# deezer/musicFPaugment

Hardware: AMD Instinct MI355X
Metric: 8s/8kHz clips/sec (STFT+UNet+peak-pick) (higher is better)
Workload: dtype bf16x3 (fp32 operands split into bf16 hi+lo, fp32 accumulate); 1 GPU; STFT(512/256,f64) -> UNet(1,1) eval forward (bf16x3 MFMA, formula weights) -> Audfprint peak-pick; 8 s / 8 kHz clips, 257x251 spectrograms; parallelism=clip-sharded x1, no data-path collective

## Files before the change

musicfpaugment_amd/csrc/unet_wd16.hip:

```cpp
#include "mfpa_common.h"
#include "mfpa_conv_tile.h"
#include "mfpa_unet_args.h"

namespace {

using namespace mfpa_tile;
using mfpa_unet::ConvArgs;

constexpr int KC = 32;

constexpr int wd16_bn(int wmw) { return 32 * (8 / wmw); }
constexpr bool wd16_persist(bool rows, int wmw, bool side, bool plain) { return wmw == 4 || (!rows && !side) || plain; }
template <int PH, int PW, bool IN16>
struct Wd16Lds {
  static constexpr int THREADS = 512;
  static constexpr int SPP = IN16 ? KC / 8 : KC / 4;
  static constexpr int HPW = PW + 2, HPH = PH + 2, HP = HPW * HPH;
  static constexpr int A_F4 = (HP * SPP + THREADS - 1) / THREADS;
  static constexpr int HPS = A_F4 * (THREADS / SPP);
  static constexpr int PLANE = ((HPS * 16 + 255) / 256) * 256;
  static constexpr int HLS = 4 * PLANE + 256;
  static constexpr int STAGE = 2 * HLS;
  static constexpr int TBL = 2 * A_F4 * THREADS;
  static constexpr int TBL_BYTES = 2 * ((HP * (KC / 4) + THREADS - 1) / THREADS) * THREADS * (int)sizeof(unsigned);
  static constexpr int RED = 2 * 256;
  static constexpr int epi_floats(int wmw) { return 2 * wd16_bn(wmw) + 64; }
  static constexpr int fixed_bytes(int wmw) { return 2 * STAGE + TBL_BYTES + epi_floats(wmw) * (int)sizeof(float); }
  __host__ __device__ static constexpr int plane_off(int hl, int kg) { return hl * HLS + kg * PLANE + (kg >> 1) * 128; }
  static_assert(TBL * (int)sizeof(unsigned) <= TBL_BYTES, "the kernel's table fits the launcher's");
};
static_assert(Wd16Lds<8, 32, false>::fixed_bytes(2) == 125184 && Wd16Lds<16, 16, false>::fixed_bytes(2) == 125184 &&
              Wd16Lds<8, 32, true>::fixed_bytes(2) == 125184 && Wd16Lds<16, 16, true>::fixed_bytes(2) == 125184, "LDS of the 128-channel tiles");
static_assert(Wd16Lds<8, 32, false>::fixed_bytes(4) == 124672 && Wd16Lds<8, 32, true>::fixed_bytes(4) == 124672, "LDS of the 64-channel tiles");


template <int CTRL>
__device__ __forceinline__ float dpp_row_add(float v) {
  return v + __int_as_float(__builtin_amdgcn_update_dpp(0, __float_as_int(v), CTRL, 0xf, 0xf, false));
}

template <int PH, int PW, bool ROWS, int WMW = 2, bool SIDE = false, bool PLAIN = false, bool IN16 = false, bool AFF16 = false>
__global__ __launch_bounds__(512, 1) void conv_wd16_kernel(ConvArgs a) {
  static_assert(!IN16 || PLAIN, "a bf16 source feeds the plain-bf16 products");
  using G = Wd16Lds<PH, PW, IN16>;
  constexpr int SPP = G::SPP, HPW = G::HPW, HP = G::HP, A_F4 = G::A_F4, HLS = G::HLS, STAGE = G::STAGE, TBL = G::TBL;
  constexpr int ESZ = IN16 ? 2 : 4;
  constexpr int THREADS = G::THREADS, BN = wd16_bn(WMW), WPXW = 256 / WMW, TAPS = 9;
  static_assert((WMW == 2 || WMW == 4) && (!ROWS || WMW == 2), "wave grid");
  constexpr int BM = PH * PW;
  static_assert(BM == 256 && (PW == 32 || PW == 16), "two waves of 128 pixels: eight 16-pixel tiles each");
  constexpr int PT = WPXW / 16;
  static_assert(A_F4 <= TAPS - 3, "one halo staging slot per tap, taps 2 .. 7");

  extern __shared__ __attribute__((aligned(16))) char smem[];
  const int tid = threadIdx.x, lane = tid & 63, wave = tid >> 6;
  const int wm = wave % WMW, wn = __builtin_amdgcn_readfirstlane(wave / WMW);
  const int p = lane & 15, g = lane >> 4;

  constexpr bool PERSIST = wd16_persist(ROWS, WMW, SIDE, PLAIN);
  const int n0 = blockIdx.y * BN;
  const int Cin = a.C0 + a.C1;
  const int nchunks = Cin / KC;
  const int ntiles = a.tiles_x * a.tiles_y * a.B;

  const int aq = tid % SPP;
  unsigned* const aoffs0 = reinterpret_cast<unsigned*>(smem + 2 * STAGE);
#pragma unroll
  for (int it = 0; it < A_F4; ++it) {
    const int pix = tid / SPP + it * (THREADS / SPP);
    const int py = pix / HPW - 1, px = pix % HPW - 1;
    aoffs0[it * THREADS + tid] = (unsigned)((py * a.W + px) * a.C0 + (KC / SPP) * aq) * (unsigned)ESZ;
    aoffs0[(A_F4 + it) * THREADS + tid] = (unsigned)(((py - a.oy1) * a.W1 + (px - a.ox1)) * a.C1 + (KC / SPP) * aq) * (unsigned)ESZ;
  }
  const unsigned clip0 = (unsigned)a.H * (unsigned)a.W * (unsigned)a.C0 * (unsigned)ESZ, clip1 = (unsigned)a.H1 * (unsigned)a.W1 * (unsigned)a.C1 * (unsigned)ESZ;
  struct Tile { int b, y0, x0p; unsigned ain; unsigned t0, t1; };
  auto make_tile = [&](int t) __attribute__((always_inline)) {
    Tile T;
    int bx = __builtin_amdgcn_readfirstlane(t);
    const int tx = bx % a.tiles_x; bx /= a.tiles_x;
    const int ty = bx % a.tiles_y; bx /= a.tiles_y;
    T.b = bx; T.y0 = ty * PH; T.x0p = tx * PW; T.ain = 0;
    T.t0 = (unsigned)((T.y0 * a.W + T.x0p) * a.C0) * (unsigned)ESZ;
    T.t1 = (unsigned)((T.y0 * a.W1 + T.x0p) * a.C1) * (unsigned)ESZ;
#pragma unroll
    for (int it = 0; it < A_F4; ++it) {
      const int pix = tid / SPP + it * (THREADS / SPP);
      const int gy = T.y0 + pix / HPW - 1, gx = T.x0p + pix % HPW - 1;
      const bool in = pix < HP && gy >= 0 && gy < a.H && gx >= 0 && gx < a.W;
      const int y1 = gy - a.oy1, x1 = gx - a.ox1;
      const bool in1 = in && y1 >= 0 && y1 < a.H1 && x1 >= 0 && x1 < a.W1;
      T.ain |= (in ? 1u : 0u) << it | (in1 ? 1u : 0u) << (8 + it);
    }
    return T;
  };
  auto clip_rsrc = [&](const float* base, int b, unsigned clip_bytes) __attribute__((always_inline)) {
    const char* pb = reinterpret_cast<const char*>(base) + (size_t)b * clip_bytes;
    return __builtin_amdgcn_make_buffer_rsrc(const_cast<char*>(pb), 0, base != nullptr ? (int)clip_bytes : 0, 0x00020000);
  };
  int tile = blockIdx.x;
  Tile S = make_tile(tile);
  int eb = S.b, ey0 = S.y0, ex0p = S.x0p;
  float* aff = reinterpret_cast<float*>(smem + 2 * STAGE + TBL * sizeof(unsigned));
  if (a.in_scale0 != nullptr) {
    for (int i = tid; i < a.C0; i += THREADS) {
      aff[i] = a.in_scale0[i];
      aff[a.C0 + i] = a.in_shift0[i];
    }
    __syncthreads();
  }
  float* const epi = aff + (a.in_scale0 ? 2 * a.C0 : 0) + (a.w1x1 ? G::RED : 0);
  for (int i = tid; i < BN; i += THREADS) {
    epi[i] = a.scale ? a.scale[n0 + i] : 1.f;
    epi[BN + i] = a.shift ? a.shift[n0 + i] : 0.f;
  }
  if (a.w1x1 != nullptr && tid < 64) epi[2 * BN + tid] = a.w1x1[tid];
  constexpr int AHALF = (A_F4 + 1) / 2, AREGS = ROWS ? AHALF : A_F4;
  f32x4 areg[AREGS];
  auto load_a_range = [&](int chunk, auto FIRST, auto COUNT) __attribute__((always_inline)) {
    constexpr int first = decltype(FIRST)::value, count = decltype(COUNT)::value;
    const int c0 = chunk * KC;
    const bool from0 = c0 < a.C0;
    const auto rs = clip_rsrc(from0 ? a.x0 : a.x1, S.b, from0 ? clip0 : clip1);
    const unsigned toff = from0 ? S.t0 + (unsigned)c0 * (unsigned)ESZ : S.t1 + (unsigned)(c0 - a.C0) * (unsigned)ESZ;
    const unsigned* ao = aoffs0 + (from0 ? 0 : A_F4 * THREADS) + tid;
#pragma unroll
    for (int it = first; it < first + count && it < A_F4; ++it)
      areg[it % AREGS] = __builtin_bit_cast(f32x4, __builtin_amdgcn_raw_buffer_load_b128(rs, (int)(ao[it * THREADS] + toff), 0, 0));
  };
  auto load_a = [&](int chunk) __attribute__((always_inline)) {
    load_a_range(chunk, std::integral_constant<int, 0>{}, std::integral_constant<int, AREGS>{});
  };
  auto preload_offsets = [&](int chunk) __attribute__((always_inline)) {
    const unsigned* ao = aoffs0 + (chunk * KC < a.C0 ? 0 : A_F4 * THREADS) + tid;
#pragma unroll
    for (int it = 0; it < A_F4; ++it) areg[it % AREGS][0] = __uint_as_float(ao[it * THREADS]);
  };
  auto load_a_pre = [&](int chunk) __attribute__((always_inline)) {
    const int c0 = chunk * KC;
    const bool from0 = c0 < a.C0;
    const auto rs = clip_rsrc(from0 ? a.x0 : a.x1, S.b, from0 ? clip0 : clip1);
    const unsigned toff = from0 ? S.t0 + (unsigned)c0 * (unsigned)ESZ : S.t1 + (unsigned)(c0 - a.C0) * (unsigned)ESZ;
#pragma unroll
    for (int it = 0; it < A_F4; ++it)
      areg[it % AREGS] = __builtin_bit_cast(f32x4, __builtin_amdgcn_raw_buffer_load_b128(rs, (int)(__float_as_uint(areg[it % AREGS][0]) + toff), 0, 0));
  };
  auto split_slot = [&](auto IT, int chunk, char* stage) __attribute__((always_inline)) {
    constexpr int it = decltype(IT)::value;
    const int pix = tid / SPP + it * (THREADS / SPP);
    const int c0 = chunk * KC;
    const bool inside = (S.ain >> ((c0 < a.C0 ? 0 : 8) + it)) & 1u;
    f32x4 v = areg[it % AREGS];
    if (!inside) v = f32x4{0.f, 0.f, 0.f, 0.f};
    if constexpr (IN16) {
      if (AFF16 && a.in_scale0 != nullptr && c0 < a.C0 && inside) {
        float f[8];
#pragma unroll
        for (int k = 0; k < 4; ++k) {
          const unsigned u = __float_as_uint(v[k]);
          f[2 * k] = __uint_as_float(u << 16);
          f[2 * k + 1] = __uint_as_float(u & 0xffff0000u);
        }
        const float* scp = aff + c0 + 8 * aq;
        const float* shp = aff + a.C0 + c0 + 8 * aq;
        const f32x4 sc0 = *reinterpret_cast<const f32x4*>(scp), sc1 = *reinterpret_cast<const f32x4*>(scp + 4);
        const f32x4 sh0 = *reinterpret_cast<const f32x4*>(shp), sh1 = *reinterpret_cast<const f32x4*>(shp + 4);
#pragma unroll
        for (int k = 0; k < 8; ++k) {
          const float y = f[k] * (k < 4 ? sc0[k & 3] : sc1[k & 3]) + (k < 4 ? sh0[k & 3] : sh1[k & 3]);
          f[k] = y > 0.f ? y : 0.f;
        }
        if (a.drop_thresh) {
          const int gy = S.y0 + pix / HPW - 1, gx = S.x0p + pix % HPW - 1;
          const unsigned long long e0 = (((unsigned long long)S.b * a.H + gy) * a.W + gx) * a.C0 + c0 + 8 * aq;
#pragma unroll
          for (int k = 0; k < 8; ++k) f[k] = mfpa_keep(a.drop_seed, a.drop_thresh, e0 + k) ? f[k] * a.drop_scale : 0.f;
        }
#pragma unroll
        for (int k = 0; k < 4; ++k) {
          bf16x2 h2;
          h2[0] = (__bf16)f[2 * k];
          h2[1] = (__bf16)f[2 * k + 1];
          v[k] = __builtin_bit_cast(float, h2);
        }
      }
      *reinterpret_cast<f32x4*>(stage + G::plane_off(0, aq) + pix * 16) = v;
      if constexpr (SIDE && AFF16) {
        const int py = pix / HPW, px = pix % HPW;
        if (a.x0_bf16 != nullptr && c0 < a.C0 && inside && py >= 1 && py <= PH && px >= 1 && px <= PW && blockIdx.y == 0) {
          const size_t e = (size_t)S.b * a.H * a.W * a.C0 + ((aoffs0[it * THREADS + tid] + S.t0) >> 1) + c0;
          *reinterpret_cast<f32x4*>(a.x0_bf16 + e) = v;
        }
      }
      return;
    }
    if (a.in_scale0 != nullptr && c0 < a.C0 && inside) {
      const f32x4 sc = *reinterpret_cast<const f32x4*>(aff + c0 + 4 * aq);
      const f32x4 sh = *reinterpret_cast<const f32x4*>(aff + a.C0 + c0 + 4 * aq);
      v = v * sc + sh;
#pragma unroll
      for (int k = 0; k < 4; ++k) v[k] = v[k] > 0.f ? v[k] : 0.f;
      if (a.drop_thresh) {
        const int gy = S.y0 + pix / HPW - 1, gx = S.x0p + pix % HPW - 1;
        const unsigned long long e0 = (((unsigned long long)S.b * a.H + gy) * a.W + gx) * a.C0 + c0 + 4 * aq;
#pragma unroll
        for (int k = 0; k < 4; ++k) v[k] = mfpa_keep(a.drop_seed, a.drop_thresh, e0 + k) ? v[k] * a.drop_scale : 0.f;
      }
    }
    bf16x4 hi, lo;
#pragma unroll
    for (int k = 0; k < 4; ++k) {
      hi[k] = (__bf16)v[k];
      lo[k] = (__bf16)(v[k] - (float)hi[k]);
    }
    char* at = stage + G::plane_off(0, aq >> 1) + pix * 16 + 8 * (aq & 1);
    *reinterpret_cast<bf16x4*>(at) = hi;
    if constexpr (!PLAIN) *reinterpret_cast<bf16x4*>(at + HLS) = lo;
    if constexpr (SIDE) {
      const int py = pix / HPW, px = pix % HPW;
      const bool interior = inside && py >= 1 && py <= PH && px >= 1 && px <= PW && blockIdx.y == 0;
      if (a.x0_bf16 != nullptr && c0 < a.C0 && interior) {
        const size_t e = (size_t)S.b * a.H * a.W * a.C0 + ((aoffs0[it * THREADS + tid] + S.t0) >> 2) + c0;
        *reinterpret_cast<bf16x4*>(a.x0_bf16 + e) = hi;
      }
      if (a.x1_bf16 != nullptr && c0 >= a.C0 && interior) {
        const size_t e = (size_t)S.b * a.H1 * a.W1 * a.C1 + ((aoffs0[(A_F4 + it) * THREADS + tid] + S.t1) >> 2) + (c0 - a.C0);
        *reinterpret_cast<bf16x4*>(a.x1_bf16 + e) = hi;
      }
    }
  };

  bf16x8 wq[3][2][2];
  auto w_frag = [&](int tap, int chunk) __attribute__((always_inline)) {
    return reinterpret_cast<const char*>(a.w) +
           ((((size_t)tap * nchunks + chunk) * (size_t)(a.Cout / 16) + (size_t)(n0 / 16 + 2 * wn)) << 11) + lane * 16;
  };
  auto load_w = [&](int chunk, int tap, auto SLOT) __attribute__((always_inline)) {
    constexpr int slot = decltype(SLOT)::value;
    const char* wb = w_frag(tap, chunk);
    wq[slot][0][0] = *reinterpret_cast<const bf16x8*>(wb);
    if constexpr (!PLAIN) wq[slot][0][1] = *reinterpret_cast<const bf16x8*>(wb + 1024);
    wq[slot][1][0] = *reinterpret_cast<const bf16x8*>(wb + 2048);
    if constexpr (!PLAIN) wq[slot][1][1] = *reinterpret_cast<const bf16x8*>(wb + 3072);
  };

  struct XFrags { bf16x8 h[4], l[4]; };
  XFrags fx0, fx1;
  const int xbase = (((wm * WPXW + p) / PW) * HPW + ((wm * WPXW + p) % PW)) * 16 + G::plane_off(0, g);
  auto tile_disp = [](int pt) { return (PW == 32) ? ((pt >> 1) * HPW + (pt & 1) * 16) * 16 : pt * HPW * 16; };
  auto read_x = [&](XFrags& f, const char* stage, int tap_off, int half) __attribute__((always_inline)) {
#pragma unroll
    for (int i = 0; i < 4; ++i) {
      const char* r = stage + xbase + tile_disp(4 * half + i) + tap_off;
      if constexpr (!PLAIN) f.l[i] = *reinterpret_cast<const bf16x8*>(r + HLS);
      f.h[i] = *reinterpret_cast<const bf16x8*>(r);
    }
  };
  floatx4 acc[2][PT];
#pragma unroll
  for (int ct = 0; ct < 2; ++ct)
#pragma unroll
    for (int pt = 0; pt < PT; ++pt) acc[ct][pt] = floatx4{0.f, 0.f, 0.f, 0.f};
  auto mfma_half = [&](const XFrags& f, const bf16x8 (&w)[2][2], int half) __attribute__((always_inline)) {
    if constexpr (!PLAIN) {
#pragma unroll
    for (int ct = 0; ct < 2; ++ct)
#pragma unroll
      for (int i = 0; i < 4; ++i) acc[ct][4 * half + i] = __builtin_amdgcn_mfma_f32_16x16x32_bf16(w[ct][1], f.h[i], acc[ct][4 * half + i], 0, 0, 0);
#pragma unroll
    for (int ct = 0; ct < 2; ++ct)
#pragma unroll
      for (int i = 0; i < 4; ++i) acc[ct][4 * half + i] = __builtin_amdgcn_mfma_f32_16x16x32_bf16(w[ct][0], f.l[i], acc[ct][4 * half + i], 0, 0, 0);
    }
#pragma unroll
    for (int ct = 0; ct < 2; ++ct)
#pragma unroll
      for (int i = 0; i < 4; ++i) acc[ct][4 * half + i] = __builtin_amdgcn_mfma_f32_16x16x32_bf16(w[ct][0], f.h[i], acc[ct][4 * half + i], 0, 0, 0);
  };
  using S0 = std::integral_constant<int, 0>;
  using S1 = std::integral_constant<int, 1>;
  constexpr int N_R = PLAIN ? 4 : 8, N_M = PLAIN ? 8 : 24;
  constexpr int N_W = PLAIN ? 2 : 4;
  auto tap_body = [&](auto TAP, int chunk) __attribute__((always_inline)) {
    constexpr int tap = decltype(TAP)::value;
    constexpr int ntap = (tap + 1) % TAPS;
    constexpr int tap_off = ((tap / 3) * HPW + (tap % 3)) * 16, ntap_off = ((ntap / 3) * HPW + (ntap % 3)) * 16;
    const int chunk_n = chunk + 1 < nchunks ? chunk + 1 : (PERSIST ? 0 : chunk);
    const char* cur = smem + (chunk & 1) * STAGE;
    const char* nxt = (tap == TAPS - 1) ? smem + ((chunk + 1) & 1) * STAGE : cur;
    read_x(fx1, cur, tap_off, 1);
    mfma_half(fx0, wq[tap % 3], 0);
    load_w((tap + 2 >= TAPS) ? chunk_n : chunk, (tap + 2) % TAPS, std::integral_constant<int, (tap + 2) % 3>{});
    pin_reads<N_M - 1, N_R>();
    constexpr int used_a = pin_read_slots(N_M - 1, N_R);
    __builtin_amdgcn_sched_group_barrier(0x008, 1, 0);
    __builtin_amdgcn_sched_group_barrier(0x020, N_W, 0);
    if constexpr (N_M - used_a - 1 > 0) __builtin_amdgcn_sched_group_barrier(0x008, N_M - used_a - 1, 0);
    __builtin_amdgcn_sched_barrier(0);
    if (tap == TAPS - 1) {
      __syncthreads();
      __builtin_amdgcn_sched_barrier(0);
    }
    if (tap == 0) load_a_pre(chunk_n);
    if (tap == TAPS - 1) preload_offsets(PERSIST ? (chunk + 2 < nchunks ? chunk + 2 : chunk + 1 < nchunks ? 0 : 1 < nchunks ? 1 : 0)
                                                 : (chunk + 2 < nchunks ? chunk + 2 : chunk + 1 < nchunks ? chunk + 1 : chunk));
    read_x(fx0, nxt, ntap_off, 0);
    mfma_half(fx1, wq[tap % 3], 1);
    if constexpr (tap >= 2 && tap - 2 < A_F4) {
      split_slot(std::integral_constant<int, tap - 2>{}, chunk_n, smem + ((chunk + 1) & 1) * STAGE);
#pragma unroll
      for (int i = 0; i < N_R; ++i) {
        __builtin_amdgcn_sched_group_barrier(0x008, 1, 0);
        __builtin_amdgcn_sched_group_barrier(0x100, 1, 0);
        __builtin_amdgcn_sched_group_barrier(0x002, 2, 0);
      }
#pragma unroll
      for (int i = 0; i < 2; ++i) {
        __builtin_amdgcn_sched_group_barrier(0x008, 2, 0);
        __builtin_amdgcn_sched_group_barrier(0x002, 4, 0);
        __builtin_amdgcn_sched_group_barrier(0x200, 1, 0);
      }
      if constexpr (N_M - N_R - 4 > 0) __builtin_amdgcn_sched_group_barrier(0x008, N_M - N_R - 4, 0);
    } else {
      pin_reads<N_M, N_R>();
      if constexpr (N_M - pin_read_slots(N_M, N_R) > 0) __builtin_amdgcn_sched_group_barrier(0x008, N_M - pin_read_slots(N_M, N_R), 0);
    }
    __builtin_amdgcn_sched_barrier(0);
  };

  auto tap_body4 = [&](auto TAP, auto PAR, int chunk) __attribute__((always_inline)) {
    constexpr int tap = decltype(TAP)::value, par = (decltype(PAR)::value + tap) & 1;
    constexpr int ntap = (tap + 1) % TAPS;
    constexpr int ntap_off = ((ntap / 3) * HPW + (ntap % 3)) * 16;
    const int chunk_n = chunk + 1 < nchunks ? chunk + 1 : 0;
    const char* cur = smem + (chunk & 1) * STAGE;
    const char* nxt = (tap == TAPS - 1) ? smem + ((chunk + 1) & 1) * STAGE : cur;
    if (tap == TAPS - 1) {
      __syncthreads();
      __builtin_amdgcn_sched_barrier(0);
    }
    if (tap == 0) load_a_pre(chunk_n);
    if (tap == TAPS - 1) preload_offsets(chunk + 2 < nchunks ? chunk + 2 : chunk + 1 < nchunks ? 0 : 1 < nchunks ? 1 : 0);
    read_x(par ? fx0 : fx1, nxt, ntap_off, 0);
    mfma_half(par ? fx1 : fx0, wq[tap % 3], 0);
    load_w((tap + 2 >= TAPS) ? chunk_n : chunk, (tap + 2) % TAPS, std::integral_constant<int, (tap + 2) % 3>{});
    if constexpr (tap >= 2 && tap - 2 < A_F4) {
      split_slot(std::integral_constant<int, tap - 2>{}, chunk_n, smem + ((chunk + 1) & 1) * STAGE);
#pragma unroll
      for (int i = 0; i < N_R; ++i) {
        __builtin_amdgcn_sched_group_barrier(0x008, 1, 0);
        __builtin_amdgcn_sched_group_barrier(0x100, 1, 0);
        __builtin_amdgcn_sched_group_barrier(0x002, 2, 0);
      }
#pragma unroll
      for (int i = 0; i < N_W; ++i) {
        if constexpr (!PLAIN) __builtin_amdgcn_sched_group_barrier(0x008, 1, 0);
        __builtin_amdgcn_sched_group_barrier(0x020, 1, 0);
        __builtin_amdgcn_sched_group_barrier(0x002, 2, 0);
      }
#pragma unroll
      for (int i = 0; i < 2; ++i) {
        __builtin_amdgcn_sched_group_barrier(0x008, 2, 0);
        __builtin_amdgcn_sched_group_barrier(0x002, 4, 0);
        __builtin_amdgcn_sched_group_barrier(0x200, 1, 0);
      }
      if constexpr (N_M - N_R - 8 > 0) __builtin_amdgcn_sched_group_barrier(0x008, N_M - N_R - 8, 0);
    } else {
#pragma unroll
      for (int i = 0; i < N_R; ++i) {
        __builtin_amdgcn_sched_group_barrier(0x008, 1, 0);
        __builtin_amdgcn_sched_group_barrier(0x100, 1, 0);
      }
#pragma unroll
      for (int i = 0; i < N_W; ++i) {
        __builtin_amdgcn_sched_group_barrier(0x008, 1, 0);
        __builtin_amdgcn_sched_group_barrier(0x020, 1, 0);
      }
      if constexpr (N_M - N_R - N_W > 0) __builtin_amdgcn_sched_group_barrier(0x008, N_M - N_R - N_W, 0);
    }
    __builtin_amdgcn_sched_barrier(0);
  };

  constexpr int R = BM / 2 / PW, HV = PW / 16;
  bf16x8 wr[2][3][2][2];
  constexpr int NU = (R + 2) * HV, NB = (PW == 32) ? 4 : 5;
  static_assert(NU % NB == 0, "static ring indices");
  auto load_wr1 = [&](int chunk, auto DX, auto PAR, auto DY) __attribute__((always_inline)) {
    constexpr int dx = decltype(DX)::value, par = decltype(PAR)::value, dy = decltype(DY)::value;
    const char* wb = w_frag(dy * 3 + dx, chunk);
    wr[par][dy][0][0] = *reinterpret_cast<const bf16x8*>(wb);
    if constexpr (!PLAIN) wr[par][dy][0][1] = *reinterpret_cast<const bf16x8*>(wb + 1024);
    wr[par][dy][1][0] = *reinterpret_cast<const bf16x8*>(wb + 2048);
    if constexpr (!PLAIN) wr[par][dy][1][1] = *reinterpret_cast<const bf16x8*>(wb + 3072);
  };
  struct XUnit { bf16x8 h, l; };
  XUnit xu[NB];
  auto read_unit = [&](XUnit& f, const char* stage, int u, int dx) __attribute__((always_inline)) {
    const char* r = stage + xbase + ((u / HV) * HPW + (u % HV) * 16 + dx) * 16;
    if constexpr (!PLAIN) f.l = *reinterpret_cast<const bf16x8*>(r + HLS);
    f.h = *reinterpret_cast<const bf16x8*>(r);
  };
  auto mfma_unit = [&](auto U, const XUnit& f, auto PAR) __attribute__((always_inline)) {
    constexpr int h = decltype(U)::value / HV, hv = decltype(U)::value % HV, par = decltype(PAR)::value;
#pragma unroll
    for (int term = PLAIN ? 2 : 0; term < 3; ++term)
#pragma unroll
      for (int dy = 0; dy < 3; ++dy) {
        if (h - dy < 0 || h - dy >= R) continue;
#pragma unroll
        for (int ct = 0; ct < 2; ++ct) {
          floatx4& c = acc[ct][(h - dy) * HV + hv];
          c = __builtin_amdgcn_mfma_f32_16x16x32_bf16(wr[par][dy][ct][term == 0 ? 1 : 0], term == 1 ? f.l : f.h, c, 0, 0, 0);
        }
      }
  };
  auto unit_mfmas = [](int u) { const int h = u / HV; int n = 0; for (int dy = 0; dy < 3; ++dy) n += (h - dy >= 0 && h - dy < R) ? 1 : 0; return n * (PLAIN ? 2 : 6); };
  constexpr int BARU = NU - NB + 1;
  constexpr int SA = NU / 2, SB = BARU - AHALF;
  static_assert(SA + AHALF < NU && SB >= 0, "staging schedule");
  auto unit_step = [&](auto U, auto DX, auto PAR, int chunk) __attribute__((always_inline)) {
    constexpr int u = decltype(U)::value, dx = decltype(DX)::value, par = decltype(PAR)::value;
    constexpr int n_m = unit_mfmas(u);
    const int chunk_n = chunk + 1 < nchunks ? chunk + 1 : (PERSIST ? 0 : chunk);
    const char* cur = smem + (chunk & 1) * STAGE;
    char* nxs = smem + ((chunk + 1) & 1) * STAGE;
    if constexpr (u == BARU && dx == 2) {
      __syncthreads();
      __builtin_amdgcn_sched_barrier(0);
    }
    constexpr int pu = u + NB - 1;
    if constexpr (pu < NU) read_unit(xu[pu % NB], cur, pu, dx);
    else read_unit(xu[pu % NB], dx == 2 ? nxs : cur, pu - NU, (dx + 1) % 3);
    mfma_unit(U, xu[u % NB], PAR);
    constexpr int split_it = dx == 1 ? u - SA : dx == 2 ? AHALF + u - SB : -1;
    constexpr bool do_split = (dx == 1 && u >= SA && u < SA + AHALF) || (dx == 2 && u >= SB && u < SB + AHALF && split_it < A_F4);
    if constexpr (u == 0 && dx == 0) load_a_range(chunk_n, std::integral_constant<int, 0>{}, std::integral_constant<int, AHALF>{});
    if constexpr (u == SA + AHALF && dx == 1) load_a_range(chunk_n, std::integral_constant<int, AHALF>{}, std::integral_constant<int, AHALF>{});
    if constexpr (u >= 1 && u <= 3) {
      if constexpr (dx < 2) load_wr1(chunk, std::integral_constant<int, (dx + 1) % 3>{}, std::integral_constant<int, par ^ 1>{}, std::integral_constant<int, u - 1>{});
      else load_wr1(chunk_n, std::integral_constant<int, 0>{}, std::integral_constant<int, par ^ 1>{}, std::integral_constant<int, u - 1>{});
    }
    if constexpr (do_split) split_slot(std::integral_constant<int, split_it>{}, chunk_n, nxs);
    __builtin_amdgcn_sched_group_barrier(0x008, 1, 0);
    __builtin_amdgcn_sched_group_barrier(0x100, PLAIN ? 1 : 2, 0);
    if constexpr (do_split && PLAIN) {
#pragma unroll
      for (int i = 1; i < n_m; ++i) {
        __builtin_amdgcn_sched_group_barrier(0x002, (24 + n_m - 2) / (n_m - 1), 0);
        __builtin_amdgcn_sched_group_barrier(0x008, 1, 0);
      }
      __builtin_amdgcn_sched_group_barrier(0x200, 1, 0);
    } else if constexpr (PLAIN && u >= 1 && u <= 3) {
      __builtin_amdgcn_sched_group_barrier(0x020, 2, 0);
      if constexpr (n_m - 1 > 0) __builtin_amdgcn_sched_group_barrier(0x008, n_m - 1, 0);
    } else if constexpr (do_split) {
      __builtin_amdgcn_sched_group_barrier(0x002, 6, 0);
#pragma unroll
      for (int i = 0; i < 4; ++i) {
        __builtin_amdgcn_sched_group_barrier(0x008, 1, 0);
        __builtin_amdgcn_sched_group_barrier(0x002, 6, 0);
      }
      __builtin_amdgcn_sched_group_barrier(0x200, 2, 0);
      if constexpr (n_m - 5 > 0) __builtin_amdgcn_sched_group_barrier(0x008, n_m - 5, 0);
    } else if constexpr (u >= 1 && u <= 3) {
#pragma unroll
      for (int i = 0; i < 4; ++i) {
        __builtin_amdgcn_sched_group_barrier(0x008, 1, 0);
        __builtin_amdgcn_sched_group_barrier(0x020, 1, 0);
      }
      if constexpr (n_m - 5 > 0) __builtin_amdgcn_sched_group_barrier(0x008, n_m - 5, 0);
    } else {
      if constexpr (n_m - 1 > 0) __builtin_amdgcn_sched_group_barrier(0x008, n_m - 1, 0);
    }
    __builtin_amdgcn_sched_barrier(0);
  };
  auto period = [&](auto DX, auto PAR, int chunk) __attribute__((always_inline)) {
    each_index<NU>(unit_step, DX, PAR, chunk);
  };

  if constexpr (ROWS) {
    f32x4 keep[AREGS];
    load_a_range(0, std::integral_constant<int, AHALF>{}, std::integral_constant<int, AHALF>{});
#pragma unroll
    for (int i = 0; i < AREGS; ++i) keep[i] = areg[i];
    load_a_range(0, std::integral_constant<int, 0>{}, std::integral_constant<int, AHALF>{});
    each_index<3>([&](auto DY) __attribute__((always_inline)) { load_wr1(0, S0{}, S0{}, DY); });
    each_index<AHALF>(split_slot, 0, smem);
#pragma unroll
    for (int i = 0; i < AREGS; ++i) areg[i] = keep[i];
    each_index<A_F4 - AHALF, AHALF>(split_slot, 0, smem);
    static_assert(A_F4 <= 2 * AHALF, "two halves of staging slots");
  } else {
    load_a(0);
    load_w(0, 0, S0{});
    load_w(0, 1, S1{});
    each_index<A_F4>(split_slot, 0, smem);
    preload_offsets(1 < nchunks ? 1 : 0);
  }
  auto epilogue = [&]() __attribute__((always_inline)) {
  #pragma unroll
    for (int ct = 0; ct < 2; ++ct) {
      const int chl = wn * 32 + ct * 16 + 4 * g;
      const f32x4 sc = *reinterpret_cast<const f32x4*>(epi + chl);
      const f32x4 sh = *reinterpret_cast<const f32x4*>(epi + BN + chl);
  #pragma unroll
      for (int pt = 0; pt < PT; ++pt)
  #pragma unroll
        for (int j = 0; j < 4; ++j) {
          float v = acc[ct][pt][j] * sc[j] + sh[j];
          if (a.relu) v = v > 0.f ? v : 0.f;
          acc[ct][pt][j] = v;
        }
    }
    if (SIDE && a.stats_part != nullptr) {
      float vm[PT];
  #pragma unroll
      for (int pt = 0; pt < PT; ++pt) {
        const int m = wm * WPXW + pt * 16 + p;
        vm[pt] = (ey0 + m / PW < a.yH && ex0p + m % PW < a.yW) ? 1.f : 0.f;
      }
      float* row = a.stats_part + ((size_t)tile * WMW + wm) * 2 * a.Cout + n0 + wn * 32 + 4 * g;
  #pragma unroll
      for (int ct = 0; ct < 2; ++ct) {
        f32x4 sv = {0.f, 0.f, 0.f, 0.f}, qv = {0.f, 0.f, 0.f, 0.f};
        if (!AFF16 && a.bz != nullptr) {
          const int ch = n0 + wn * 32 + ct * 16 + 4 * g;
          const f32x4 bsc = *reinterpret_cast<const f32x4*>(a.bz_scale + ch), bsh = *reinterpret_cast<const f32x4*>(a.bz_shift + ch);
          const f32x4 bmu = *reinterpret_cast<const f32x4*>(a.bz_mean + ch), bis = *reinterpret_cast<const f32x4*>(a.bz_invstd + ch);
          f32x4 zzs[PT];
          auto zoff = [&](int pt) __attribute__((always_inline)) {
            const int m = wm * WPXW + pt * 16 + p;
            const int gy = min(ey0 + m / PW, a.yH - 1), gx = min(ex0p + m % PW, a.yW - 1);
            return (((size_t)eb * a.yH + gy) * a.yW + gx) * (size_t)a.Cout + ch;
          };
          if (a.bz16) {
            f32x2 raw[PT];
  #pragma unroll
            for (int pt = 0; pt < PT; ++pt) raw[pt] = *reinterpret_cast<const f32x2*>(reinterpret_cast<const __bf16*>(a.bz) + zoff(pt));
  #pragma unroll
            for (int pt = 0; pt < PT; ++pt) {
              const unsigned u0 = __float_as_uint(raw[pt][0]), u1 = __float_as_uint(raw[pt][1]);
              zzs[pt] = f32x4{__uint_as_float(u0 << 16), __uint_as_float(u0 & 0xffff0000u), __uint_as_float(u1 << 16), __uint_as_float(u1 & 0xffff0000u)};
            }
          } else {
  #pragma unroll
            for (int pt = 0; pt < PT; ++pt) zzs[pt] = *reinterpret_cast<const f32x4*>(a.bz + zoff(pt));
          }
  #pragma unroll
          for (int pt = 0; pt < PT; ++pt) {
            const f32x4 zz = zzs[pt];
  #pragma unroll
            for (int j = 0; j < 4; ++j) {
              const float gg = (zz[j] * bsc[j] + bsh[j] > 0.f) ? acc[ct][pt][j] * vm[pt] : 0.f;
              sv[j] += gg;
              qv[j] += gg * ((zz[j] - bmu[j]) * bis[j]);
            }
          }
        } else {
  #pragma unroll
        for (int pt = 0; pt < PT; ++pt)
  #pragma unroll
          for (int j = 0; j < 4; ++j) {
            const float v = acc[ct][pt][j] * vm[pt];
            sv[j] += v;
            qv[j] += v * v;
          }
        }
  #pragma unroll
        for (int j = 0; j < 4; ++j) {
          sv[j] = dpp_row_add<0x118>(dpp_row_add<0x114>(dpp_row_add<0x112>(dpp_row_add<0x111>(sv[j]))));
          qv[j] = dpp_row_add<0x118>(dpp_row_add<0x114>(dpp_row_add<0x112>(dpp_row_add<0x111>(qv[j]))));
        }
        if (p == 15) {
          *reinterpret_cast<f32x4*>(row + ct * 16) = sv;
          *reinterpret_cast<f32x4*>(row + a.Cout + ct * 16) = qv;
        }
      }
    }
    if (a.y != nullptr || (SIDE && IN16 && a.y_bf16 != nullptr)) {
      char* yb = reinterpret_cast<char*>(a.y + (size_t)eb * a.yH * a.yW * a.Cout);
  #pragma unroll
      for (int pt = 0; pt < PT; ++pt) {
        const int m = wm * WPXW + pt * 16 + p;
        const int gy = ey0 + m / PW, gx = ex0p + m % PW;
        if (gy < a.yH && gx < a.yW) {
          char* yp = yb + (((unsigned)gy * (unsigned)a.yW + (unsigned)gx) * (unsigned)a.Cout + (unsigned)(n0 + wn * 32 + 4 * g)) * 4u;
          if (a.y != nullptr) {
  #pragma unroll
          for (int ct = 0; ct < 2; ++ct) {
            f32x4 o;
  #pragma unroll
            for (int j = 0; j < 4; ++j) o[j] = acc[ct][pt][j];
            *reinterpret_cast<f32x4*>(yp + ct * 64) = o;
          }
          }
          if (SIDE && a.y_bf16 != nullptr) {
            __bf16* hp = a.y_bf16 + (((size_t)eb * a.yH + gy) * a.yW + gx) * (size_t)a.Cout + n0 + wn * 32 + 4 * g;
  #pragma unroll
            for (int ct = 0; ct < 2; ++ct) {
              bf16x4 h;
  #pragma unroll
              for (int j = 0; j < 4; ++j) h[j] = (__bf16)acc[ct][pt][j];
              *reinterpret_cast<bf16x4*>(hp + ct * 16) = h;
            }
          }
        }
      }
    }
    if (a.y_pool != nullptr) {
      const int Ho = a.H / 2, Wo = a.W / 2;
      constexpr int ROWSTEP = (PW == 32) ? 2 : 1;
  #pragma unroll
      for (int ct = 0; ct < 2; ++ct)
  #pragma unroll
        for (int pt = 0; pt < PT; ++pt) {
          const int row = pt / ROWSTEP;
          if (row & 1) continue;
          f32x4 v;
  #pragma unroll
          for (int j = 0; j < 4; ++j) {
            const float t = fmaxf(acc[ct][pt][j], acc[ct][pt + ROWSTEP][j]);
            const float o = __int_as_float(__builtin_amdgcn_update_dpp(0, __float_as_int(t), 0xB1, 0xf, 0xf, true));
            v[j] = fmaxf(t, o);
          }
          const int m = wm * WPXW + pt * 16 + p;
          const int py = (ey0 + m / PW) / 2, px = (ex0p + m % PW) / 2;
          if (!(p & 1) && py < Ho && px < Wo)
            *reinterpret_cast<f32x4*>(a.y_pool + (((size_t)eb * Ho + py) * Wo + px) * a.Cout + n0 + wn * 32 + ct * 16 + 4 * g) = v;
        }
    }
  
    if constexpr (WMW == 4) {
      if (a.w1x1 != nullptr) {
        float* red = reinterpret_cast<float*>(smem + 2 * STAGE + TBL * sizeof(unsigned)) + (a.in_scale0 ? 2 * a.C0 : 0);
        const f32x4 w0 = *reinterpret_cast<const f32x4*>(epi + 2 * BN + wn * 32 + 4 * g);
        const f32x4 w1 = *reinterpret_cast<const f32x4*>(epi + 2 * BN + wn * 32 + 16 + 4 * g);
  #pragma unroll
        for (int pt = 0; pt < PT; ++pt) {
          float v = 0.f;
  #pragma unroll
          for (int j = 0; j < 4; ++j) v += acc[0][pt][j] * w0[j] + acc[1][pt][j] * w1[j];
          v += __shfl_xor(v, 16);
          v += __shfl_xor(v, 32);
          if (g == 0) red[wn * 256 + wm * WPXW + pt * 16 + p] = v;
        }
        __syncthreads();
        if (tid < 256) {
          const int gy = ey0 + tid / PW, gx = ex0p + tid % PW;
          if (gy < a.H && gx < a.W) a.y1x1[((size_t)eb * a.H + gy) * a.W + gx] = red[tid] + red[256 + tid] + a.b1x1;
        }
        __syncthreads();
      }
    }
  };

  __syncthreads();
  if constexpr (ROWS) {
#pragma unroll
    for (int u = 0; u < NB - 1; ++u) read_unit(xu[u], smem, u, 0);
  } else {
    read_x(fx0, smem, 0, 0);
  }
  for (;;) {
    const int tile_n = tile + (int)gridDim.x;
    const bool has_next = PERSIST && tile_n < ntiles;
    const Tile N = PERSIST ? make_tile(has_next ? tile_n : tile) : S;
    if constexpr (ROWS) {
      using D0 = std::integral_constant<int, 0>;
      using D1 = std::integral_constant<int, 1>;
      using D2 = std::integral_constant<int, 2>;
      for (int chunk = 0; chunk < nchunks; chunk += 2) {
        period(D0{}, S0{}, chunk);
        period(D1{}, S1{}, chunk);
        period(D2{}, S0{}, chunk);
        if (PERSIST && chunk + 2 >= nchunks) S = N;
        period(D0{}, S1{}, chunk + 1);
        period(D1{}, S0{}, chunk + 1);
        period(D2{}, S1{}, chunk + 1);
      }
    } else if constexpr (WMW == 4) {
      for (int chunk = 0; chunk < nchunks; chunk += 2) {
        each_index<TAPS>(tap_body4, S0{}, chunk);
        if (chunk + 2 >= nchunks) S = N;
        each_index<TAPS>(tap_body4, S1{}, chunk + 1);
      }
    } else {
      for (int chunk = 0; chunk < nchunks; ++chunk) {
        if (PERSIST && chunk + 1 >= nchunks) S = N;
        each_index<TAPS>(tap_body, chunk);
      }
    }
    epilogue();
    if (!has_next) break;
    tile = tile_n; eb = S.b; ey0 = S.y0; ex0p = S.x0p;
#pragma unroll
    for (int ct = 0; ct < 2; ++ct)
#pragma unroll
      for (int pt = 0; pt < PT; ++pt) acc[ct][pt] = floatx4{0.f, 0.f, 0.f, 0.f};
  }
}

}

namespace mfpa_unet {

const int CONV_WD16_ROWS = 512;
void conv_wd16_tile(int W, int Cout, mfpa_conv_route* t) {
  t->wmw = Cout % 128 ? 4 : 2; t->bn = 32 * (8 / t->wmw);
  t->pw = (t->wmw == 2 && W <= 16) ? 16 : 32; t->ph = 256 / t->pw;
}

template <int PH, int PW, bool ROWS, int WMW, bool SIDE, bool PLAIN, bool IN16, bool AFF16>
int launch_wd16(ConvArgs& a, hipStream_t s) {
  using G = Wd16Lds<PH, PW, IN16>;
  const size_t lds = (size_t)G::fixed_bytes(WMW) +
                     (a.in_scale0 ? (size_t)2 * a.C0 * sizeof(float) : 0) +
                     (a.w1x1 ? G::RED * sizeof(float) : 0);
  dim3 grid((unsigned)((long long)a.tiles_x * a.tiles_y * a.B), (unsigned)(a.Cout / wd16_bn(WMW)));
  if constexpr (wd16_persist(ROWS, WMW, SIDE, PLAIN)) {
    const int cus = mfpa_current_device_cus();
    const unsigned per = (unsigned)((cus > 0 ? cus : 256) / (int)grid.y);
    if (per >= 1 && grid.x > per) grid.x = per;
  }
  hipLaunchKernelGGL((conv_wd16_kernel<PH, PW, ROWS, WMW, SIDE, PLAIN, IN16, AFF16>), grid, dim3(G::THREADS), lds, s, a);
  MFPA_CHECK_LAUNCH();
  return MFPA_OK;
}
#define MFPA_WD16_INSTANTIATE(...) template int launch_wd16<__VA_ARGS__>(ConvArgs&, hipStream_t);
MFPA_WD16_FORMS(MFPA_WD16_INSTANTIATE)

}
```

Baseline: 5043 clips/s.

## Make rows-mode wd16 conv persistent with lean register usage for tile indices

Turns on persistent tile looping for the non-side rows variant, which previously launched one block per tile. To hold down the VGPR pressure this adds, a LEAN mode rebuilds the lane-derived values (tid, p, g, wm) on demand through mbcnt, with an asm barrier stopping the compiler from keeping them live. It also builds the next tile only at the swap point rather than ahead of it, and derives the dropout element index from the stored offset table. The trade is extra recomputation and a later next-tile setup in exchange for block-launch savings and less register pressure.

```diff
diff --git a/musicfpaugment_amd/csrc/unet_wd16.hip b/musicfpaugment_amd/csrc/unet_wd16.hip
--- a/musicfpaugment_amd/csrc/unet_wd16.hip
+++ b/musicfpaugment_amd/csrc/unet_wd16.hip
@@ -10,7 +10,8 @@
 constexpr int KC = 32;
 
 constexpr int wd16_bn(int wmw) { return 32 * (8 / wmw); }
-constexpr bool wd16_persist(bool rows, int wmw, bool side, bool plain) { return wmw == 4 || (!rows && !side) || plain; }
+constexpr bool wd16_persist(bool rows, int wmw, bool side, bool plain) { return wmw == 4 || !side || plain; }
+constexpr bool wd16_lean(bool rows, int wmw, bool side, bool plain) { return rows && wmw == 2 && !side && !plain; }
 template <int PH, int PW, bool IN16>
 struct Wd16Lds {
   static constexpr int THREADS = 512;
@@ -54,8 +55,15 @@
 
   extern __shared__ __attribute__((aligned(16))) char smem[];
   const int tid = threadIdx.x, lane = tid & 63, wave = tid >> 6;
-  const int wm = wave % WMW, wn = __builtin_amdgcn_readfirstlane(wave / WMW);
-  const int p = lane & 15, g = lane >> 4;
+  int wm = wave % WMW, wn = __builtin_amdgcn_readfirstlane(wave / WMW);
+  int p = lane & 15, g = lane >> 4;
+  constexpr bool LEAN = wd16_lean(ROWS, WMW, SIDE, PLAIN);
+  const int wave_s = __builtin_amdgcn_readfirstlane(wave);
+  auto lane_now = [&]() __attribute__((always_inline)) {
+    int l = __builtin_amdgcn_mbcnt_hi(~0u, __builtin_amdgcn_mbcnt_lo(~0u, 0u));
+    asm volatile("" : "+v"(l));
+    return l;
+  };
 
   constexpr bool PERSIST = wd16_persist(ROWS, WMW, SIDE, PLAIN);
   const int n0 = blockIdx.y * BN;
@@ -82,9 +90,10 @@
     T.b = bx; T.y0 = ty * PH; T.x0p = tx * PW; T.ain = 0;
     T.t0 = (unsigned)((T.y0 * a.W + T.x0p) * a.C0) * (unsigned)ESZ;
     T.t1 = (unsigned)((T.y0 * a.W1 + T.x0p) * a.C1) * (unsigned)ESZ;
+    const int lt = LEAN ? wave_s * 64 + lane_now() : tid;
 #pragma unroll
     for (int it = 0; it < A_F4; ++it) {
-      const int pix = tid / SPP + it * (THREADS / SPP);
+      const int pix = lt / SPP + it * (THREADS / SPP);
       const int gy = T.y0 + pix / HPW - 1, gx = T.x0p + pix % HPW - 1;
       const bool in = pix < HP && gy >= 0 && gy < a.H && gx >= 0 && gx < a.W;
       const int y1 = gy - a.oy1, x1 = gx - a.ox1;
@@ -200,8 +209,13 @@
 #pragma unroll
       for (int k = 0; k < 4; ++k) v[k] = v[k] > 0.f ? v[k] : 0.f;
       if (a.drop_thresh) {
-        const int gy = S.y0 + pix / HPW - 1, gx = S.x0p + pix % HPW - 1;
-        const unsigned long long e0 = (((unsigned long long)S.b * a.H + gy) * a.W + gx) * a.C0 + c0 + 4 * aq;
+        unsigned long long e0;
+        if constexpr (LEAN) {
+          e0 = (unsigned long long)S.b * a.H * a.W * a.C0 + ((aoffs0[it * THREADS + tid] + S.t0) >> 2) + c0;
+        } else {
+          const int gy = S.y0 + pix / HPW - 1, gx = S.x0p + pix % HPW - 1;
+          e0 = (((unsigned long long)S.b * a.H + gy) * a.W + gx) * a.C0 + c0 + 4 * aq;
+        }
 #pragma unroll
         for (int k = 0; k < 4; ++k) v[k] = mfpa_keep(a.drop_seed, a.drop_thresh, e0 + k) ? v[k] * a.drop_scale : 0.f;
       }
@@ -663,7 +677,8 @@
   for (;;) {
     const int tile_n = tile + (int)gridDim.x;
     const bool has_next = PERSIST && tile_n < ntiles;
-    const Tile N = PERSIST ? make_tile(has_next ? tile_n : tile) : S;
+    Tile N = S;
+    if constexpr (PERSIST && !LEAN) N = make_tile(has_next ? tile_n : tile);
     if constexpr (ROWS) {
       using D0 = std::integral_constant<int, 0>;
       using D1 = std::integral_constant<int, 1>;
@@ -672,7 +687,10 @@
         period(D0{}, S0{}, chunk);
         period(D1{}, S1{}, chunk);
         period(D2{}, S0{}, chunk);
-        if (PERSIST && chunk + 2 >= nchunks) S = N;
+        if (PERSIST && chunk + 2 >= nchunks) {
+          if constexpr (LEAN) S = make_tile(has_next ? tile_n : tile);
+          else S = N;
+        }
         period(D0{}, S1{}, chunk + 1);
         period(D1{}, S0{}, chunk + 1);
         period(D2{}, S1{}, chunk + 1);
@@ -688,6 +706,10 @@
         if (PERSIST && chunk + 1 >= nchunks) S = N;
         each_index<TAPS>(tap_body, chunk);
       }
+    }
+    if constexpr (LEAN) {
+      const int el = lane_now();
+      p = el & 15; g = el >> 4; wm = wave_s % WMW;
     }
     epilogue();
     if (!has_next) break;
```

Result: no change. 5068 clips/s (median of 6 runs) (+0.5%).
